# 2gunsu/monocon-pytorch

Measured on AMD Instinct MI355X. Metric: images/sec (384x1280) fwd+bwd, higher is better.
Workload: dtype f32 (f16x2); 1 GPU; train step B=32/GPU 3x384x1280 (configs[2] shape, fp32 values, mode f16x2); global_batch=32, parallelism=dp1, precision_mode=f16x2

## Files before the change

### monocon-pytorch_amd/csrc/conv_thin.hip

```cpp
#include "conv_mfma.h"
#include "train.h"

#ifndef THIN_OCC
#define THIN_OCC 2
#endif
#ifndef THIN_MT_UNROLL
#define THIN_MT_UNROLL 1
#endif
namespace mc {

typedef _Float16 f16x8 __attribute__((ext_vector_type(8)));
typedef _Float16 f16x4 __attribute__((ext_vector_type(4)));
typedef float f32x4v __attribute__((ext_vector_type(4)));

namespace {
constexpr int TR = 8, TW = 64;
constexpr int IR = TR + 2, IP = TW + 2;
constexpr int PLANE = IR * IP * 16;
constexpr int ITEMS = IR * IP * 4;
constexpr int NI = (ITEMS + 255) / 256;
}

template <int NTN>
__global__ __launch_bounds__(256, THIN_OCC) void conv_thin16_kernel(const ConvArgs a) {
    constexpr int CIN = 16;
    __shared__ __attribute__((aligned(16))) unsigned char lds[4 * PLANE];
    const int tid = threadIdx.x, lane = tid & 63;
    const int wave = __builtin_amdgcn_readfirstlane(tid >> 6);
    const int li = lane & 15, kq = lane >> 4;
    const int half = kq & 1, tsel = kq >> 1;

    const int ex = f16_scale_exp(amax_read(a.amax_in[0])), ew = f16_scale_exp(*a.amax_w);
    const float x_scale = exp2i(ex), w_scale = exp2i(ew);
    const float omul = exp2i(-ex) * exp2i(-ew);
    const bool lazy = a.src[0].la != nullptr;
    f32x4 lzA = {0.f, 0.f, 0.f, 0.f}, lzB = lzA;
    if (lazy) {
        lzA = reinterpret_cast<const f32x4 *>(a.src[0].la)[tid & 3];
        lzB = reinterpret_cast<const f32x4 *>(a.src[0].lb)[tid & 3];
#pragma unroll
        for (int j = 0; j < 4; ++j) { lzA[j] *= x_scale; lzB[j] *= x_scale; }
    }
    const unsigned x_bytes = (unsigned)(a.Hin * a.Win * CIN) * 4u;
    unsigned okm = 0u;

    f16x8 bw[5][2][NTN];
#pragma unroll
    for (int s = 0; s < 5; ++s) {
        const int tap = 2 * s + tsel;
#pragma unroll
        for (int nt = 0; nt < NTN; ++nt) {
            f16x8 h8, l8;
#pragma unroll
            for (int c4 = 0; c4 < 2; ++c4) {
                f32x4 w = {0.f, 0.f, 0.f, 0.f};
                if (tap < 9)
                    w = *reinterpret_cast<const f32x4 *>(a.wpk + ((size_t)(tap * (CIN / 4) + half * 2 + c4) * a.CoutP + nt * 16 + li) * 4);
#pragma unroll
                for (int j = 0; j < 4; ++j) {
                    const float ws = w[j] * w_scale;
                    const _Float16 hh = (_Float16)ws;
                    h8[c4 * 4 + j] = hh;
                    l8[c4 * 4 + j] = (_Float16)(ws - (float)hh);
                }
            }
            bw[s][0][nt] = h8;
            bw[s][1][nt] = l8;
        }
    }

    float sc[NTN], bi[NTN], sh[NTN];
    bool nok[NTN];
#pragma unroll
    for (int nt = 0; nt < NTN; ++nt) {
        const int n = nt * 16 + li;
        nok[nt] = n < a.Cout;
        sc[nt] = (a.scale && nok[nt]) ? a.scale[n] : 1.f;
        bi[nt] = (a.bias && nok[nt]) ? a.bias[n] : 0.f;
        sh[nt] = (a.stat_shift && nok[nt]) ? a.stat_shift[n] : 0.f;
    }
    const bool do_stats = a.stats != nullptr, has_res = a.res != nullptr;
    const float floor_v = a.relu ? 0.f : -__builtin_inff();
    float vmax = 0.f;
    const bool bm = a.bm_y != nullptr;
    const int bm_relu = a.bm_relu;
    float ma[NTN], mb[NTN];
#pragma unroll
    for (int nt = 0; nt < NTN; ++nt) {
        ma[nt] = (bm && bm_relu == 2 && nok[nt]) ? a.bm_a[nt * 16 + li] : 0.f;
        mb[nt] = (bm && bm_relu == 2 && nok[nt]) ? a.bm_b[nt * 16 + li] : 0.f;
    }

    int s_off[NI], s_dst[NI];
#pragma unroll
    for (int i = 0; i < NI; ++i) {
        const int e = tid + 256 * i;
        const int c4 = e & 3, px = (e >> 2) % IP, row = (e >> 2) / IP;
        s_off[i] = ((row * a.Win + px) * CIN + c4 * 4) * 4;
        s_dst[i] = e < ITEMS ? ((c4 >> 1) * PLANE) + (row * IP + px) * 16 + (c4 & 1) * 8 : -1;
    }

    const int tiles_per_img = (a.Hout + TR - 1) / TR;
    const int nstrips = (a.Wout + TW - 1) / TW;
    for (int tile = xcd_order(blockIdx.x, gridDim.x); tile < a.B * tiles_per_img; tile += gridDim.x) {
        const int img = tile / tiles_per_img, oy0 = (tile - img * tiles_per_img) * TR;
        const __amdgpu_buffer_rsrc_t r_x = make_rsrc(a.src[0].p + (size_t)img * a.Hin * a.Win * CIN, (unsigned)(a.Hin * a.Win * CIN) * 4u);
        __amdgpu_buffer_rsrc_t r_out[2], r_res[2];
#pragma unroll
        for (int q = 0; q < 2; ++q) {
            const int oy = oy0 + 2 * wave + q;
            const bool ok = oy < a.Hout;
            const size_t row = (size_t)img * a.Hout + (ok ? oy : 0);
            r_out[q] = make_rsrc(a.out + row * a.Wout * a.out_ld, ok ? (unsigned)(a.Wout * a.out_ld) * 4u : 0u);
            r_res[q] = make_rsrc(has_res ? a.res + row * a.Wout * a.res_ld : a.out, (has_res && ok) ? (unsigned)(a.Wout * a.res_ld) * 4u : 0u);
        }
        float ssum[2][NTN], ssq[2][NTN];
#pragma unroll
        for (int q = 0; q < 2; ++q)
#pragma unroll
            for (int nt = 0; nt < NTN; ++nt) ssum[q][nt] = ssq[q][nt] = 0.f;

        f32x4 pre[NI];
        const int band_off = ((oy0 - 1) * a.Win - 1) * CIN * 4;
        auto fetch = [&](int strip) {
            const int x0 = strip * TW - 1, so = band_off + strip * TW * CIN * 4;
            okm = 0u;
            if (strip > 0 && x0 + IP <= a.Win) {
#pragma unroll
                for (int i = 0; i < NI; ++i) {
                    const int vo = s_dst[i] >= 0 ? s_off[i] + so : BUF_OOB;
                    pre[i] = buf_load4(r_x, vo, 0);
                    if (lazy) okm |= ((unsigned)vo < x_bytes ? 1u : 0u) << i;
                }
            } else {
#pragma unroll
                for (int i = 0; i < NI; ++i) {
                    const int px = ((s_dst[i] % PLANE) >> 4) % IP;
                    const bool ok = s_dst[i] >= 0 && (unsigned)(x0 + px) < (unsigned)a.Win;
                    const int vo = ok ? s_off[i] + so : BUF_OOB;
                    pre[i] = buf_load4(r_x, vo, 0);
                    if (lazy) okm |= ((unsigned)vo < x_bytes ? 1u : 0u) << i;
                }
            }
        };
        auto store = [&]() {
#pragma unroll
            for (int i = 0; i < NI; ++i) {
                if (256 * (i + 1) > ITEMS && s_dst[i] < 0) continue;
                f16x4 h4, l4;
                const float cap = ((okm >> i) & 1u) ? __builtin_inff() : 0.f;
#pragma unroll
                for (int j = 0; j < 4; ++j) {
                    const float xs = lazy ? lazy_act(pre[i][j], lzA[j], lzB[j], cap) : pre[i][j] * x_scale;
                    const _Float16 hh = (_Float16)xs;
                    h4[j] = hh;
                    l4[j] = (_Float16)(xs - (float)hh);
                }
                *reinterpret_cast<f16x4 *>(lds + s_dst[i]) = h4;
                *reinterpret_cast<f16x4 *>(lds + 2 * PLANE + s_dst[i]) = l4;
            }
        };

        fetch(0);
        for (int strip = 0; strip < nstrips; ++strip) {
            __syncthreads();
            store();
            __syncthreads();
            if (strip + 1 < nstrips) fetch(strip + 1);
            const int sx0 = strip * TW;
#pragma unroll
            for (int q = 0; q < 2; ++q) {
                const int trow = 2 * wave + q;
#pragma unroll THIN_MT_UNROLL
                for (int mt = 0; mt < TW / 16; ++mt) {
                    const int x0 = sx0 + mt * 16;
                    if (x0 >= a.Wout) break;
                    f32x4v acc[NTN], accm[NTN];
#pragma unroll
                    for (int nt = 0; nt < NTN; ++nt) { acc[nt] = f32x4v{0.f, 0.f, 0.f, 0.f}; accm[nt] = f32x4v{0.f, 0.f, 0.f, 0.f}; }
                    const bool rok = oy0 + trow < a.Hout;
                    float ybm[NTN][4], zbm[NTN][4];
                    if (bm) {
#pragma unroll
                        for (int nt = 0; nt < NTN; ++nt) {
                            const size_t at0 = (((size_t)img * a.Hout + (rok ? oy0 + trow : 0)) * a.Wout + x0 + 4 * kq) * a.Cout + nt * 16 + li;
#pragma unroll
                            for (int e = 0; e < 4; ++e) {
                                const bool ld = rok && nok[nt];
                                ybm[nt][e] = ld ? a.bm_y[at0 + (size_t)e * a.Cout] : 0.f;
                                zbm[nt][e] = (ld && bm_relu == 1) ? a.bm_z[at0 + (size_t)e * a.Cout] : 1.f;
                            }
                        }
                    }
#pragma unroll
                    for (int s = 0; s < 5; ++s) {
                        const int tap = 2 * s + tsel;
                        const int r = tap / 3, c = tap - 3 * r;
                        f16x8 ah = {0, 0, 0, 0, 0, 0, 0, 0}, al = ah;
                        if (tap < 9) {
                            const unsigned char *p = lds + half * PLANE + ((trow + r) * IP + mt * 16 + li + c) * 16;
                            ah = *reinterpret_cast<const f16x8 *>(p);
                            al = *reinterpret_cast<const f16x8 *>(p + 2 * PLANE);
                        }
#pragma unroll
                        for (int nt = 0; nt < NTN; ++nt) {
                            accm[nt] = __builtin_amdgcn_mfma_f32_16x16x32_f16(al, bw[s][0][nt], accm[nt], 0, 0, 0);
                            accm[nt] = __builtin_amdgcn_mfma_f32_16x16x32_f16(ah, bw[s][1][nt], accm[nt], 0, 0, 0);
                            acc[nt] = __builtin_amdgcn_mfma_f32_16x16x32_f16(ah, bw[s][0][nt], acc[nt], 0, 0, 0);
                        }
                    }
#pragma unroll
                    for (int nt = 0; nt < NTN; ++nt) {
                        const int n = nt * 16 + li;
                        const int v_out = nok[nt] ? ((4 * kq) * a.out_ld + a.out_coff + n) * 4 : BUF_OOB;
                        const int v_res = nok[nt] ? ((4 * kq) * a.res_ld + n) * 4 : BUF_OOB;
                        float rv[4];
                        if (has_res) {
#pragma unroll
                            for (int e = 0; e < 4; ++e) rv[e] = buf_load1(r_res[q], v_res, (x0 + e) * a.res_ld * 4);
                        }
#pragma unroll
                        for (int e = 0; e < 4; ++e) {
                            float v = ((accm[nt][e] + acc[nt][e]) * omul) * sc[nt] + bi[nt];
                            if (has_res) v += rv[e];
                            if (bm) {
                                if (rok && nok[nt]) {
                                    const float yv = ybm[nt][e];
                                    const bool on = bm_relu == 0 || (bm_relu == 1 ? zbm[nt][e] > 0.f : fmaf(yv, ma[nt], mb[nt]) > 0.f);
                                    v = on ? v : 0.f;
                                    ssum[q][nt] += v;
                                    ssq[q][nt] = fmaf(v, yv, ssq[q][nt]);
                                }
                            } else if (do_stats) {
                                const float d = v - sh[nt];
                                ssum[q][nt] += d;
                                ssq[q][nt] += d * d;
                            }
                            v = fmaxf(v, floor_v);
                            vmax = fmaxf(vmax, (nok[nt] && oy0 + trow < a.Hout) ? fabsf(v) : 0.f);
                            buf_store1(v, r_out[q], v_out, (x0 + e) * a.out_ld * 4);
                        }
                    }
                }
            }
        }
        if (do_stats) {
#pragma unroll
            for (int q = 0; q < 2; ++q) {
                const int oy = oy0 + 2 * wave + q;
                if (oy >= a.Hout) continue;
#pragma unroll
                for (int nt = 0; nt < NTN; ++nt) {
                    float s1 = ssum[q][nt], s2 = ssq[q][nt];
                    s1 += __shfl_xor(s1, 16); s2 += __shfl_xor(s2, 16);
                    s1 += __shfl_xor(s1, 32); s2 += __shfl_xor(s2, 32);
                    if (kq == 0 && nok[nt]) {
                        float *dst = a.stats + (((size_t)img * a.Hout + oy) * a.CoutP + nt * 16 + li) * 2;
                        dst[0] = s1;
                        dst[1] = s2;
                    }
                }
            }
        }
    }
    if (a.amax_out) amax_update_wave(a.amax_out, vmax);
}

bool conv_thin_ok(const ConvArgs &a, int ks, int stride) {
#ifdef MC_NO_CONV_THIN
    return false;
#endif
    return a.prec == 3 && ks == 3 && stride == 1 && a.nsrc == 1 && a.Cin == 16 && a.Cout == 16 && a.amax_in[0] && a.amax_w &&
           a.Wout % 16 == 0 && a.Hout == a.Hin && a.Wout == a.Win && a.CoutP >= 16;
}

hipError_t launch_conv_thin(const ConvArgs &a, hipStream_t st) {
    const int tiles = a.B * ((a.Hout + TR - 1) / TR);
    hipLaunchKernelGGL((conv_thin16_kernel<1>), dim3(tiles < 4096 ? tiles : 4096), dim3(256), 0, st, a);
    return hipGetLastError();
}


struct DgradS2Args {
    const float *dy;
    const float *w;
    float *out;
    int B, H, W, CinTotal, c_off, accumulate;
    const unsigned *amax_dy, *amax_w;
};
namespace {
constexpr int DR = 4, DW = 32;
constexpr int DIR_ = DR + 1, DIP = DW + 1;
constexpr int DPLANE = DIR_ * DIP * 16;
}
template <int KS, int NT>
__global__ __launch_bounds__(256, KS == 1 ? 2 : 1) void dgrad_s2_thin_kernel(const DgradS2Args a) {
    constexpr int CY = 32 * KS, CX = 16 * NT, NOCT = 4 * KS;
    constexpr int DITEMS = DIR_ * DIP * (CY / 4), DNI = (DITEMS + 255) / 256;
    __shared__ __attribute__((aligned(16))) unsigned char lds[2 * NOCT * DPLANE];
    const int tid = threadIdx.x, lane = tid & 63;
    const int wave = __builtin_amdgcn_readfirstlane(tid >> 6);
    const int li = lane & 15, kq = lane >> 4;
    const int nt = wave % NT, row0 = (wave / NT) * NT;
    const int ex = f16_scale_exp(amax_read(a.amax_dy)), ew = f16_scale_exp(*a.amax_w);
    const float x_scale = exp2i(ex), w_scale = exp2i(ew), omul = exp2i(-ex) * exp2i(-ew);
    f16x8 bw[9][KS][2];
// ... 94 lines not shown
                                const int voff = j < a.W ? ((2 * j + px) * CX + 16 * nt + li) * 4 : BUF_OOB;
                                float v = (accm[e] + acc[e]) * omul;
                                if (a.accumulate) v += buf_load1(r_out[rr][py], voff, 0);
                                buf_store1(v, r_out[rr][py], voff, 0);
                            }
                        }
                    }
                }
            }
        }
    }
}
bool dgrad_s2_thin_ok(int prec, int ks, int stride, int dyC, int srcC, int CinTotal, int c_off, const unsigned *amax_dy,
                      const unsigned *amax_w, int H, int W) {
    const bool shape = dyC == 32 && srcC == 16;
    return prec == 3 && ks == 3 && stride == 2 && shape && c_off >= 0 && c_off + srcC <= CinTotal && amax_dy && amax_w &&
           (size_t)H * W * dyC * 4 < (1ull << 31) && (size_t)4 * W * srcC * 4 < (1ull << 31);
}
hipError_t launch_dgrad_s2_thin(const float *dy, int B, int H, int W, int dyC, const float *w_master, int CinTotal, int c_off, float *out,
                                int accumulate, const unsigned *amax_dy, const unsigned *amax_w, hipStream_t st) {
    DgradS2Args a;
    a.dy = dy; a.w = w_master; a.out = out; a.B = B; a.H = H; a.W = W; a.CinTotal = CinTotal; a.c_off = c_off;
    a.accumulate = accumulate; a.amax_dy = amax_dy; a.amax_w = amax_w;
    const int tiles = B * ((H + DR - 1) / DR);
    const int srcC = dyC / 2;
    prof_last = {1, 2.0 * B * H * W * (double)dyC * srcC * 9.0, 4.0 * ((double)B * H * W * dyC + (double)B * 4 * H * W * srcC * (accumulate ? 2 : 1))};
    if (dyC != 32) return hipErrorInvalidValue;
    hipLaunchKernelGGL((dgrad_s2_thin_kernel<1, 1>), dim3(tiles < 4096 ? tiles : 4096), dim3(256), 0, st, a);
    return hipGetLastError();
}

namespace {
constexpr int WT_XT = 128, WT_P = 152, WT_ROWS = 6;
constexpr int WT_PLANE = 16 * WT_ROWS * WT_P * 2;
typedef unsigned u32x4 __attribute__((ext_vector_type(4)));
typedef _Float16 f16x2 __attribute__((ext_vector_type(2)));
}

__global__ __launch_bounds__(256) void wgrad_thin16_kernel(const WgradArgs a) {
    extern __shared__ __attribute__((aligned(16))) unsigned char wsm[];
    unsigned char *win = wsm;
    float (*red)[64] = reinterpret_cast<float (*)[64]>(wsm + 2 * WT_PLANE);
    const int tid = threadIdx.x, lane = tid & 63;
    const int wave = __builtin_amdgcn_readfirstlane(tid >> 6);
    const int g = lane >> 4, j = lane & 15;
    const int ex = f16_scale_exp(amax_read(a.amax_x[0])), ed = f16_scale_exp(amax_read(a.amax_dy));
    const float x_scale = exp2i(ex), d_scale = exp2i(ed), omul = exp2i(-ex) * exp2i(-ed);
    const int H = a.Hout, W = a.Wout;
    const bool lazy = a.src[0].la != nullptr;
    f32x4 lzA = {0.f, 0.f, 0.f, 0.f}, lzB = lzA;
    if (lazy) {
        lzA = reinterpret_cast<const f32x4 *>(a.src[0].la)[tid & 3];
        lzB = reinterpret_cast<const f32x4 *>(a.src[0].lb)[tid & 3];
#pragma unroll
        for (int q = 0; q < 4; ++q) { lzA[q] *= x_scale; lzB[q] *= x_scale; }
    }
    const unsigned x_bytes = (unsigned)(a.Hin * a.Win * 16) * 4u;
    unsigned okm = 0u;

    f32x4v acc[9], accm[9];
#pragma unroll
    for (int t = 0; t < 9; ++t) { acc[t] = f32x4v{0.f, 0.f, 0.f, 0.f}; accm[t] = f32x4v{0.f, 0.f, 0.f, 0.f}; }
    const int va = (8 * g * 16 + j) * 4;
    const int boff = ((j * WT_ROWS + wave) * WT_P + 8 * g) * 2;

    constexpr int NITEM = WT_ROWS * (WT_P / 2) * 4, NIW = (NITEM + 255) / 256;
    int w_off[NIW], w_dst[NIW];
#pragma unroll
    for (int i = 0; i < NIW; ++i) {
        const int e = tid + 256 * i, c4 = e & 3, pr = (e >> 2) % (WT_P / 2), row = (e >> 2) / (WT_P / 2);
        w_off[i] = ((row * a.Win + 2 * pr) * 16 + c4 * 4) * 4;
        w_dst[i] = e < NITEM ? ((c4 * 4 * WT_ROWS + row) * WT_P + 2 * pr) * 2 : -1;
    }
    const int tiles_x = (W + WT_XT - 1) / WT_XT, tiles_y = (H + 3) / 4;
    const int ntiles = a.B * tiles_y * tiles_x;
    f32x4 pv[NIW][2];
    auto fetch = [&](int tl) {
        const int b = tl / (tiles_y * tiles_x), rem = tl - b * tiles_y * tiles_x;
        const int y0 = (rem / tiles_x) * 4, x0 = (rem % tiles_x) * WT_XT;
        const __amdgpu_buffer_rsrc_t r_x = make_rsrc(a.src[0].p + (size_t)b * a.Hin * a.Win * 16, (unsigned)(a.Hin * a.Win * 16) * 4u);
        const int so = ((y0 - 1) * a.Win + x0 - 1) * 64;
        okm = 0u;
#pragma unroll
        for (int i = 0; i < NIW; ++i) {
            const int col = x0 - 1 + ((w_dst[i] >> 1) % WT_P);
            const bool live = w_dst[i] >= 0;
            const int vo0 = (live && col >= 0 && col < a.Win) ? w_off[i] + so : BUF_OOB;
            const int vo1 = (live && col + 1 >= 0 && col + 1 < a.Win) ? w_off[i] + so + 64 : BUF_OOB;
            pv[i][0] = buf_load4(r_x, vo0, 0);
            pv[i][1] = buf_load4(r_x, vo1, 0);
            if (lazy) okm |= (((unsigned)vo0 < x_bytes ? 1u : 0u) | ((unsigned)vo1 < x_bytes ? 2u : 0u)) << (2 * i);
        }
    };
    float araw[WT_XT / 32][8];
    auto fetch_dy = [&](int tl, float (&dst)[WT_XT / 32][8]) {
        const int b = tl / (tiles_y * tiles_x), rem = tl - b * tiles_y * tiles_x;
        const int y = (rem / tiles_x) * 4 + wave, x0 = (rem % tiles_x) * WT_XT;
        const __amdgpu_buffer_rsrc_t r_dy =
            make_rsrc(a.dy + ((size_t)b * H + (y < H ? y : 0)) * W * a.dy_ld, y < H ? (unsigned)(W * a.dy_ld) * 4u : 0u);
#pragma unroll
        for (int G = 0; G < WT_XT / 32; ++G)
#pragma unroll
            for (int t = 0; t < 8; ++t) dst[G][t] = buf_load1(r_dy, va + t * 64, (x0 + G * 32) * 64);
// ... 108 lines not shown
```

### monocon-pytorch_amd/csrc/stem_f16.hip

```cpp
#include "conv_mfma.h"
#include "kernels.h"

#ifndef STEM_MT_UNROLL
#define STEM_MT_UNROLL 1
#endif
namespace mc {

typedef _Float16 f16x8 __attribute__((ext_vector_type(8)));
typedef _Float16 f16x4 __attribute__((ext_vector_type(4)));
typedef float f32x4v __attribute__((ext_vector_type(4)));

namespace {
constexpr int SR = 8, SW = 64;
constexpr int SIR = SR + 6, SIP = 72;
constexpr int SPIX = SIR * SIP;
constexpr int SNI = (SPIX + 255) / 256;
}

__global__ __launch_bounds__(256) void stem_f16_kernel(const float *__restrict__ img, int B, int H, int W,
                                                       const float *__restrict__ wpk ,
                                                       const float *__restrict__ scale, const float *__restrict__ shift,
                                                       float *__restrict__ out, int relu, unsigned *__restrict__ amax_out,
                                                       float *__restrict__ stats ,
                                                       const float *__restrict__ stat_shift,
                                                       unsigned *__restrict__ img_amax ) {
    __shared__ __attribute__((aligned(16))) unsigned char lds[2 * SPIX * 8];
    __shared__ unsigned s_max;
    const int tid = threadIdx.x, lane = tid & 63;
    const int wave = __builtin_amdgcn_readfirstlane(tid >> 6);
    const int li = lane & 15, kq = lane >> 4;
    const int tiles_y = (H + SR - 1) / SR, nstrips = (W + SW - 1) / SW;
    const int bt = xcd_order(blockIdx.x, gridDim.x);
    const int b = bt / tiles_y;
    const int ty0 = (bt % tiles_y) * SR;

    float wv[7][8];
    float wmax = 0.f;
#pragma unroll
    for (int r = 0; r < 7; ++r)
#pragma unroll
        for (int p = 0; p < 2; ++p)
#pragma unroll
            for (int c = 0; c < 4; ++c) {
                const int s = 2 * kq + p;
                const float w = (c < 3 && s < 7) ? wpk[((c * 7 + r) * 7 + s) * 16 + li] : 0.f;
                wv[r][p * 4 + c] = w;
                wmax = fmaxf(wmax, fabsf(w));
            }
#pragma unroll
    for (int o = 32; o > 0; o >>= 1) wmax = fmaxf(wmax, __shfl_xor(wmax, o));
    const int ew = f16_scale_exp(__builtin_bit_cast(unsigned, wmax));
    const float w_scale = exp2i(ew);
    f16x8 bw[7][2];
#pragma unroll
    for (int r = 0; r < 7; ++r)
#pragma unroll
        for (int j = 0; j < 8; ++j) {
            const float ws = wv[r][j] * w_scale;
            const _Float16 hh = (_Float16)ws;
            bw[r][0][j] = hh;
            bw[r][1][j] = (_Float16)(ws - (float)hh);
        }

    const float sc = scale[li], sf = shift[li];
    const float sh = (stats && stat_shift) ? stat_shift[li] : 0.f;
    float vmax = 0.f;
    float ssum[2] = {0.f, 0.f}, ssq[2] = {0.f, 0.f};

    float xin[SNI][3];
    auto fetch = [&](int strip) {
        const int tx0 = strip * SW;
#pragma unroll
        for (int i = 0; i < SNI; ++i) {
            const int e = tid + 256 * i;
            const int ly = e / SIP, lx = e - ly * SIP;
            const int y = ty0 - 3 + ly, x = tx0 - 3 + lx;
            const bool ok = e < SPIX && y >= 0 && y < H && x >= 0 && x < W;
#pragma unroll
            for (int c = 0; c < 3; ++c) xin[i][c] = ok ? img[(((size_t)b * 3 + c) * H + y) * W + x] : 0.f;
        }
    };
    fetch(0);
    for (int strip = 0; strip < nstrips; ++strip) {
        const int tx0 = strip * SW;
        float xmax = 0.f;
#pragma unroll
        for (int i = 0; i < SNI; ++i)
#pragma unroll
            for (int c = 0; c < 3; ++c) xmax = fmaxf(xmax, fabsf(xin[i][c]));
        if (tid == 0) s_max = 0u;
        __syncthreads();
        {
            const unsigned bits = __builtin_bit_cast(unsigned, xmax);
            if (bits != 0u && bits < 0x7f800000u) atomicMax(&s_max, bits);
        }
        __syncthreads();
        const int ex = f16_scale_exp(s_max);
        const float x_scale = exp2i(ex);
        const float omul = exp2i(-ex) * exp2i(-ew);
        if (img_amax && tid == 0) amax_commit(img_amax, s_max);
// ... 1 lines not shown
        for (int i = 0; i < SNI; ++i) {
            const int e = tid + 256 * i;
            if (e >= SPIX) continue;
            f16x4 h4, l4;
#pragma unroll
            for (int c = 0; c < 4; ++c) {
                const float xs = c < 3 ? xin[i][c] * x_scale : 0.f;
                const _Float16 hh = (_Float16)xs;
                h4[c] = hh;
                l4[c] = (_Float16)(xs - (float)hh);
            }
            *reinterpret_cast<f16x4 *>(lds + e * 8) = h4;
            *reinterpret_cast<f16x4 *>(lds + SPIX * 8 + e * 8) = l4;
        }
        __syncthreads();
        if (strip + 1 < nstrips) fetch(strip + 1);
#pragma unroll
        for (int q = 0; q < 2; ++q) {
            const int trow = 2 * wave + q, y = ty0 + trow;
            if (y >= H) continue;
            float *orow = out + ((size_t)b * H + y) * W * 16;
#pragma unroll STEM_MT_UNROLL
            for (int mt = 0; mt < SW / 16; ++mt) {
                const int x0 = tx0 + mt * 16;
                if (x0 >= W) break;
                f32x4v acc = {0.f, 0.f, 0.f, 0.f}, accm = {0.f, 0.f, 0.f, 0.f};
#pragma unroll
                for (int r = 0; r < 7; ++r) {
                    const unsigned char *p = lds + ((trow + r) * SIP + mt * 16 + li + 2 * kq) * 8;
                    const f16x4 h0 = *reinterpret_cast<const f16x4 *>(p), h1 = *reinterpret_cast<const f16x4 *>(p + 8);
                    const f16x4 l0 = *reinterpret_cast<const f16x4 *>(p + SPIX * 8), l1 = *reinterpret_cast<const f16x4 *>(p + SPIX * 8 + 8);
                    const f16x8 ah = {h0[0], h0[1], h0[2], h0[3], h1[0], h1[1], h1[2], h1[3]};
                    const f16x8 al = {l0[0], l0[1], l0[2], l0[3], l1[0], l1[1], l1[2], l1[3]};
                    accm = __builtin_amdgcn_mfma_f32_16x16x32_f16(al, bw[r][0], accm, 0, 0, 0);
                    accm = __builtin_amdgcn_mfma_f32_16x16x32_f16(ah, bw[r][1], accm, 0, 0, 0);
                    acc = __builtin_amdgcn_mfma_f32_16x16x32_f16(ah, bw[r][0], acc, 0, 0, 0);
                }
#pragma unroll
                for (int e = 0; e < 4; ++e) {
                    const int x = x0 + 4 * kq + e;
                    float v = fmaf((accm[e] + acc[e]) * omul, sc, sf);
                    if (relu) v = fmaxf(v, 0.f);
                    if (x < W) {
                        orow[(size_t)x * 16 + li] = v;
                        vmax = fmaxf(vmax, fabsf(v));
                        const float d = v - sh;
                        ssum[q] += d;
                        ssq[q] = fmaf(d, d, ssq[q]);
                    }
                }
            }
        }
    }
    if (stats) {
#pragma unroll
        for (int q = 0; q < 2; ++q) {
            const int y = ty0 + 2 * wave + q;
            float s1 = ssum[q], s2 = ssq[q];
            s1 += __shfl_xor(s1, 16); s2 += __shfl_xor(s2, 16);
            s1 += __shfl_xor(s1, 32); s2 += __shfl_xor(s2, 32);
            if (kq == 0 && y < H) {
                float *dst = stats + (((size_t)b * H + y) * 16 + li) * 2;
                dst[0] = s1;
                dst[1] = s2;
            }
        }
    }
    if (amax_out) amax_update_wave(amax_out, vmax);
}

hipError_t launch_stem_f16(const float *img, int B, int H, int W, const float *wpk, const float *scale, const float *shift,
                           float *out, hipStream_t st, int relu, unsigned *amax_out, float *stats, const float *stat_shift,
                           unsigned *img_amax) {
    const int tiles = (H + SR - 1) / SR;
    hipLaunchKernelGGL(stem_f16_kernel, dim3(B * tiles), dim3(256), 0, st, img, B, H, W, wpk, scale, shift, out, relu, amax_out, stats,
                       stat_shift, img_amax);
    return hipGetLastError();
}


namespace {
constexpr int GW_XT = 128, GW_P = 144, GW_ROWS = 10;
typedef unsigned u32x4 __attribute__((ext_vector_type(4)));
}

template <bool FUSED>
__global__ __launch_bounds__(256) void stem_wgrad_f16_kernel(const float *__restrict__ img, const float *__restrict__ dy, int B,
                                                             int H, int W, float *__restrict__ partial,
                                                             const unsigned *__restrict__ img_amax,
                                                             const unsigned *__restrict__ dy_amax,
                                                             const float *__restrict__ ybn, const float *__restrict__ coef,
                                                             const unsigned *__restrict__ y_amax) {
    constexpr int PLANE_B = 3 * GW_ROWS * GW_P * 2;
    __shared__ __attribute__((aligned(16))) unsigned char win[2 * PLANE_B];
    __shared__ float red[14 * 4][64];
    const int tid = threadIdx.x, lane = tid & 63;
    const int wave = __builtin_amdgcn_readfirstlane(tid >> 6);
    const int g = lane >> 4, j = lane & 15;
    float cP = 0.f, cQ = 0.f, cR = 0.f;
    int ed;
    if constexpr (FUSED) {
        const f32x4v cf = reinterpret_cast<const f32x4v *>(coef)[j];
        cP = cf[0]; cQ = cf[1]; cR = cf[2];
        float mP = fabsf(cP), mQ = fabsf(cQ), mR = fabsf(cR);
#pragma unroll
        for (int o = 8; o > 0; o >>= 1) {
            mP = fmaxf(mP, __shfl_xor(mP, o)); mQ = fmaxf(mQ, __shfl_xor(mQ, o)); mR = fmaxf(mR, __shfl_xor(mR, o));
        }
        const float bound = mP * __builtin_bit_cast(float, amax_read(dy_amax)) + mQ * __builtin_bit_cast(float, amax_read(y_amax)) + mR;
        ed = f16_scale_exp(__builtin_bit_cast(unsigned, bound));
    } else {
        ed = f16_scale_exp(amax_read(dy_amax));
    }
    const int ex = f16_scale_exp(amax_read(img_amax));
    const float x_scale = exp2i(ex), d_scale = exp2i(ed), omul = exp2i(-ex) * exp2i(-ed);
    int boff[2];
#pragma unroll
    for (int grp = 0; grp < 2; ++grp) {
        const int cr = grp * 16 + j, c = cr / 7, r = cr - 7 * c;
        boff[grp] = cr < 21 ? ((c * GW_ROWS + wave + r) * GW_P + 8 * g) * 2 : 0;
    }
    f32x4v acc[2][7], accm[2][7];
#pragma unroll
    for (int grp = 0; grp < 2; ++grp)
#pragma unroll
        for (int sft = 0; sft < 7; ++sft) { acc[grp][sft] = f32x4v{0.f, 0.f, 0.f, 0.f}; accm[grp][sft] = f32x4v{0.f, 0.f, 0.f, 0.f}; }
    const int va = (8 * g * 16 + j) * 4;
    const int tiles_x = (W + GW_XT - 1) / GW_XT, tiles_y = (H + 3) / 4;
    const int ntiles = B * tiles_y * tiles_x;
    constexpr int NPAIR = 3 * GW_ROWS * (GW_P / 2), NIW = (NPAIR + 255) / 256;
    int w_c[NIW], w_rr[NIW], w_col[NIW];
#pragma unroll
    for (int i = 0; i < NIW; ++i) {
        const int e = tid + 256 * i, row = e / (GW_P / 2);
        w_c[i] = e < NPAIR ? row / GW_ROWS : -1;
        w_rr[i] = row % GW_ROWS;
        w_col[i] = (e - row * (GW_P / 2)) * 2;
    }
    float pv[NIW][2];
    auto fetch = [&](int tl) {
        const int b = tl / (tiles_y * tiles_x), rem = tl - b * tiles_y * tiles_x;
        const int y0 = (rem / tiles_x) * 4, x0 = (rem % tiles_x) * GW_XT;
#pragma unroll
        for (int i = 0; i < NIW; ++i) {
            const int gy = y0 - 3 + w_rr[i], gx = x0 - 3 + w_col[i];
            const bool rok = w_c[i] >= 0 && gy >= 0 && gy < H;
            const float *src = img + (((size_t)b * 3 + (rok ? w_c[i] : 0)) * H + (rok ? gy : 0)) * W;
            pv[i][0] = (rok && gx >= 0 && gx < W) ? src[gx] : 0.f;
            pv[i][1] = (rok && gx + 1 >= 0 && gx + 1 < W) ? src[gx + 1] : 0.f;
        }
    };
    if ((int)blockIdx.x < ntiles) fetch(blockIdx.x);
    for (int tl = blockIdx.x; tl < ntiles; tl += gridDim.x) {
        const int b = tl / (tiles_y * tiles_x), rem = tl - b * tiles_y * tiles_x;
        const int y0 = (rem / tiles_x) * 4, x0 = (rem % tiles_x) * GW_XT;
        __syncthreads();
#pragma unroll
        for (int i = 0; i < NIW; ++i) {
            if (w_c[i] < 0) continue;
            const float s0 = pv[i][0] * x_scale, s1 = pv[i][1] * x_scale;
            const _Float16 h0 = (_Float16)s0, h1 = (_Float16)s1;
            typedef _Float16 f16x2 __attribute__((ext_vector_type(2)));
            const f16x2 hp = {h0, h1}, lp = {(_Float16)(s0 - (float)h0), (_Float16)(s1 - (float)h1)};
            const int off = ((w_c[i] * GW_ROWS + w_rr[i]) * GW_P + w_col[i]) * 2;
            *reinterpret_cast<f16x2 *>(win + off) = hp;
            *reinterpret_cast<f16x2 *>(win + PLANE_B + off) = lp;
        }
        __syncthreads();
        if (tl + (int)gridDim.x < ntiles) fetch(tl + gridDim.x);
        const int y = y0 + wave;
// ... 99 lines not shown
```

Before: 678.4 images/sec.

## Transpose MFMA operands in thin16/stem convs for vectorized 128-bit epilogue stores

Swaps the A/B operands of the MFMA calls in the thin 16-channel conv and the stem conv, so each lane's accumulator holds 4 consecutive output channels of one pixel instead of 4 pixels of one channel. The epilogue can then use a single 128-bit buffer store and load per tile for output, residual and backward-mask inputs, replacing four scalar strided accesses. Per-channel scale, bias and stat accumulators become 4-wide, and the stats reduction moves to a 16-lane shuffle tree. The change also trims the wgrad window fetch to the columns actually used, raises stem occupancy via launch bounds, and adds alignment guards on out_ld, out_coff and res_ld. It costs more registers for the per-channel vectors and extra shuffles in the stats reduction.

```diff
diff --git a/monocon-pytorch_amd/csrc/conv_thin.hip b/monocon-pytorch_amd/csrc/conv_thin.hip
--- a/monocon-pytorch_amd/csrc/conv_thin.hip
+++ b/monocon-pytorch_amd/csrc/conv_thin.hip
@@ -14,6 +14,9 @@
 typedef float f32x4v __attribute__((ext_vector_type(4)));
 
 namespace {
+__device__ __forceinline__ void buf_store4(f32x4 v, __amdgpu_buffer_rsrc_t r, int voff, int soff) {
+    __builtin_amdgcn_raw_buffer_store_b128(__builtin_bit_cast(i32x4, v), r, voff, soff, 0);
+}
 constexpr int TR = 8, TW = 64;
 constexpr int IR = TR + 2, IP = TW + 2;
 constexpr int PLANE = IR * IP * 16;
@@ -69,27 +72,32 @@
         }
     }
 
-    float sc[NTN], bi[NTN], sh[NTN];
+    float sc[NTN][4], bi[NTN][4], sh[NTN][4];
     bool nok[NTN];
 #pragma unroll
     for (int nt = 0; nt < NTN; ++nt) {
-        const int n = nt * 16 + li;
-        nok[nt] = n < a.Cout;
-        sc[nt] = (a.scale && nok[nt]) ? a.scale[n] : 1.f;
-        bi[nt] = (a.bias && nok[nt]) ? a.bias[n] : 0.f;
-        sh[nt] = (a.stat_shift && nok[nt]) ? a.stat_shift[n] : 0.f;
+        const int n0 = nt * 16 + 4 * kq;
+        nok[nt] = n0 + 3 < a.Cout;
+#pragma unroll
+        for (int e = 0; e < 4; ++e) {
+            sc[nt][e] = (a.scale && nok[nt]) ? a.scale[n0 + e] : 1.f;
+            bi[nt][e] = (a.bias && nok[nt]) ? a.bias[n0 + e] : 0.f;
+            sh[nt][e] = (a.stat_shift && nok[nt]) ? a.stat_shift[n0 + e] : 0.f;
+        }
     }
     const bool do_stats = a.stats != nullptr, has_res = a.res != nullptr;
     const float floor_v = a.relu ? 0.f : -__builtin_inff();
     float vmax = 0.f;
     const bool bm = a.bm_y != nullptr;
     const int bm_relu = a.bm_relu;
-    float ma[NTN], mb[NTN];
-#pragma unroll
-    for (int nt = 0; nt < NTN; ++nt) {
-        ma[nt] = (bm && bm_relu == 2 && nok[nt]) ? a.bm_a[nt * 16 + li] : 0.f;
-        mb[nt] = (bm && bm_relu == 2 && nok[nt]) ? a.bm_b[nt * 16 + li] : 0.f;
-    }
+    float ma[NTN][4], mb[NTN][4];
+#pragma unroll
+    for (int nt = 0; nt < NTN; ++nt)
+#pragma unroll
+        for (int e = 0; e < 4; ++e) {
+            ma[nt][e] = (bm && bm_relu == 2 && nok[nt]) ? a.bm_a[nt * 16 + 4 * kq + e] : 0.f;
+            mb[nt][e] = (bm && bm_relu == 2 && nok[nt]) ? a.bm_b[nt * 16 + 4 * kq + e] : 0.f;
+        }
 
     int s_off[NI], s_dst[NI];
 #pragma unroll
@@ -114,11 +122,11 @@
             r_out[q] = make_rsrc(a.out + row * a.Wout * a.out_ld, ok ? (unsigned)(a.Wout * a.out_ld) * 4u : 0u);
             r_res[q] = make_rsrc(has_res ? a.res + row * a.Wout * a.res_ld : a.out, (has_res && ok) ? (unsigned)(a.Wout * a.res_ld) * 4u : 0u);
         }
-        float ssum[2][NTN], ssq[2][NTN];
+        f32x4 ssum[2][NTN], ssq[2][NTN];
 #pragma unroll
         for (int q = 0; q < 2; ++q)
 #pragma unroll
-            for (int nt = 0; nt < NTN; ++nt) ssum[q][nt] = ssq[q][nt] = 0.f;
+            for (int nt = 0; nt < NTN; ++nt) ssum[q][nt] = ssq[q][nt] = f32x4{0.f, 0.f, 0.f, 0.f};
 
         f32x4 pre[NI];
         const int band_off = ((oy0 - 1) * a.Win - 1) * CIN * 4;
@@ -179,17 +187,14 @@
 #pragma unroll
                     for (int nt = 0; nt < NTN; ++nt) { acc[nt] = f32x4v{0.f, 0.f, 0.f, 0.f}; accm[nt] = f32x4v{0.f, 0.f, 0.f, 0.f}; }
                     const bool rok = oy0 + trow < a.Hout;
-                    float ybm[NTN][4], zbm[NTN][4];
+                    f32x4 ybm[NTN], zbm[NTN];
                     if (bm) {
 #pragma unroll
                         for (int nt = 0; nt < NTN; ++nt) {
-                            const size_t at0 = (((size_t)img * a.Hout + (rok ? oy0 + trow : 0)) * a.Wout + x0 + 4 * kq) * a.Cout + nt * 16 + li;
-#pragma unroll
-                            for (int e = 0; e < 4; ++e) {
-                                const bool ld = rok && nok[nt];
-                                ybm[nt][e] = ld ? a.bm_y[at0 + (size_t)e * a.Cout] : 0.f;
-                                zbm[nt][e] = (ld && bm_relu == 1) ? a.bm_z[at0 + (size_t)e * a.Cout] : 1.f;
-                            }
+                            const size_t at0 = (((size_t)img * a.Hout + (rok ? oy0 + trow : 0)) * a.Wout + x0 + li) * a.Cout + nt * 16 + 4 * kq;
+                            const bool ld = rok && nok[nt];
+                            ybm[nt] = ld ? *reinterpret_cast<const f32x4 *>(a.bm_y + at0) : f32x4{0.f, 0.f, 0.f, 0.f};
+                            zbm[nt] = (ld && bm_relu == 1) ? *reinterpret_cast<const f32x4 *>(a.bm_z + at0) : f32x4{1.f, 1.f, 1.f, 1.f};
                         }
                     }
 #pragma unroll
@@ -204,42 +209,40 @@
                         }
 #pragma unroll
                         for (int nt = 0; nt < NTN; ++nt) {
-                            accm[nt] = __builtin_amdgcn_mfma_f32_16x16x32_f16(al, bw[s][0][nt], accm[nt], 0, 0, 0);
-                            accm[nt] = __builtin_amdgcn_mfma_f32_16x16x32_f16(ah, bw[s][1][nt], accm[nt], 0, 0, 0);
-                            acc[nt] = __builtin_amdgcn_mfma_f32_16x16x32_f16(ah, bw[s][0][nt], acc[nt], 0, 0, 0);
+                            accm[nt] = __builtin_amdgcn_mfma_f32_16x16x32_f16(bw[s][0][nt], al, accm[nt], 0, 0, 0);
+                            accm[nt] = __builtin_amdgcn_mfma_f32_16x16x32_f16(bw[s][1][nt], ah, accm[nt], 0, 0, 0);
+                            acc[nt] = __builtin_amdgcn_mfma_f32_16x16x32_f16(bw[s][0][nt], ah, acc[nt], 0, 0, 0);
                         }
                     }
 #pragma unroll
                     for (int nt = 0; nt < NTN; ++nt) {
-                        const int n = nt * 16 + li;
-                        const int v_out = nok[nt] ? ((4 * kq) * a.out_ld + a.out_coff + n) * 4 : BUF_OOB;
-                        const int v_res = nok[nt] ? ((4 * kq) * a.res_ld + n) * 4 : BUF_OOB;
-                        float rv[4];
-                        if (has_res) {
-#pragma unroll
-                            for (int e = 0; e < 4; ++e) rv[e] = buf_load1(r_res[q], v_res, (x0 + e) * a.res_ld * 4);
-                        }
+                        const int n0 = nt * 16 + 4 * kq;
+                        const int v_out = nok[nt] ? (li * a.out_ld + a.out_coff + n0) * 4 : BUF_OOB;
+                        const int v_res = nok[nt] ? (li * a.res_ld + n0) * 4 : BUF_OOB;
+                        f32x4 rv = {0.f, 0.f, 0.f, 0.f}, o;
+                        if (has_res) rv = buf_load4(r_res[q], v_res, x0 * a.res_ld * 4);
 #pragma unroll
                         for (int e = 0; e < 4; ++e) {
-                            float v = ((accm[nt][e] + acc[nt][e]) * omul) * sc[nt] + bi[nt];
+                            float v = ((accm[nt][e] + acc[nt][e]) * omul) * sc[nt][e] + bi[nt][e];
                             if (has_res) v += rv[e];
                             if (bm) {
                                 if (rok && nok[nt]) {
                                     const float yv = ybm[nt][e];
-                                    const bool on = bm_relu == 0 || (bm_relu == 1 ? zbm[nt][e] > 0.f : fmaf(yv, ma[nt], mb[nt]) > 0.f);
+                                    const bool on = bm_relu == 0 || (bm_relu == 1 ? zbm[nt][e] > 0.f : fmaf(yv, ma[nt][e], mb[nt][e]) > 0.f);
                                     v = on ? v : 0.f;
-                                    ssum[q][nt] += v;
-                                    ssq[q][nt] = fmaf(v, yv, ssq[q][nt]);
+                                    ssum[q][nt][e] += v;
+                                    ssq[q][nt][e] = fmaf(v, yv, ssq[q][nt][e]);
                                 }
                             } else if (do_stats) {
-                                const float d = v - sh[nt];
-                                ssum[q][nt] += d;
-                                ssq[q][nt] += d * d;
+                                const float d = v - sh[nt][e];
+                                ssum[q][nt][e] += d;
+                                ssq[q][nt][e] += d * d;
                             }
                             v = fmaxf(v, floor_v);
                             vmax = fmaxf(vmax, (nok[nt] && oy0 + trow < a.Hout) ? fabsf(v) : 0.f);
-                            buf_store1(v, r_out[q], v_out, (x0 + e) * a.out_ld * 4);
+                            o[e] = v;
                         }
+                        buf_store4(o, r_out[q], v_out, x0 * a.out_ld * 4);
                     }
                 }
             }
@@ -251,13 +254,16 @@
                 if (oy >= a.Hout) continue;
 #pragma unroll
                 for (int nt = 0; nt < NTN; ++nt) {
-                    float s1 = ssum[q][nt], s2 = ssq[q][nt];
-                    s1 += __shfl_xor(s1, 16); s2 += __shfl_xor(s2, 16);
-                    s1 += __shfl_xor(s1, 32); s2 += __shfl_xor(s2, 32);
-                    if (kq == 0 && nok[nt]) {
-                        float *dst = a.stats + (((size_t)img * a.Hout + oy) * a.CoutP + nt * 16 + li) * 2;
-                        dst[0] = s1;
-                        dst[1] = s2;
+#pragma unroll
+                    for (int e = 0; e < 4; ++e) {
+                        float s1 = ssum[q][nt][e], s2 = ssq[q][nt][e];
+#pragma unroll
+                        for (int o = 1; o < 16; o <<= 1) { s1 += __shfl_xor(s1, o); s2 += __shfl_xor(s2, o); }
+                        if (li == 0 && nok[nt]) {
+                            float *dst = a.stats + (((size_t)img * a.Hout + oy) * a.CoutP + nt * 16 + 4 * kq + e) * 2;
+                            dst[0] = s1;
+                            dst[1] = s2;
+                        }
                     }
                 }
             }
@@ -271,7 +277,8 @@
     return false;
 #endif
     return a.prec == 3 && ks == 3 && stride == 1 && a.nsrc == 1 && a.Cin == 16 && a.Cout == 16 && a.amax_in[0] && a.amax_w &&
-           a.Wout % 16 == 0 && a.Hout == a.Hin && a.Wout == a.Win && a.CoutP >= 16;
+           a.Wout % 16 == 0 && a.Hout == a.Hin && a.Wout == a.Win && a.CoutP >= 16 &&
+           a.out_ld % 4 == 0 && a.out_coff % 4 == 0 && (!a.res || a.res_ld % 4 == 0);
 }
 
 hipError_t launch_conv_thin(const ConvArgs &a, hipStream_t st) {
@@ -432,6 +439,7 @@
 
 namespace {
 constexpr int WT_XT = 128, WT_P = 152, WT_ROWS = 6;
+constexpr int WT_USED = 130;
 constexpr int WT_PLANE = 16 * WT_ROWS * WT_P * 2;
 typedef unsigned u32x4 __attribute__((ext_vector_type(4)));
 typedef _Float16 f16x2 __attribute__((ext_vector_type(2)));
@@ -464,11 +472,11 @@
     const int va = (8 * g * 16 + j) * 4;
     const int boff = ((j * WT_ROWS + wave) * WT_P + 8 * g) * 2;
 
-    constexpr int NITEM = WT_ROWS * (WT_P / 2) * 4, NIW = (NITEM + 255) / 256;
+    constexpr int NITEM = WT_ROWS * (WT_USED / 2) * 4, NIW = (NITEM + 255) / 256;
     int w_off[NIW], w_dst[NIW];
 #pragma unroll
     for (int i = 0; i < NIW; ++i) {
-        const int e = tid + 256 * i, c4 = e & 3, pr = (e >> 2) % (WT_P / 2), row = (e >> 2) / (WT_P / 2);
+        const int e = tid + 256 * i, c4 = e & 3, pr = (e >> 2) % (WT_USED / 2), row = (e >> 2) / (WT_USED / 2);
         w_off[i] = ((row * a.Win + 2 * pr) * 16 + c4 * 4) * 4;
         w_dst[i] = e < NITEM ? ((c4 * 4 * WT_ROWS + row) * WT_P + 2 * pr) * 2 : -1;
     }
diff --git a/monocon-pytorch_amd/csrc/stem_f16.hip b/monocon-pytorch_amd/csrc/stem_f16.hip
--- a/monocon-pytorch_amd/csrc/stem_f16.hip
+++ b/monocon-pytorch_amd/csrc/stem_f16.hip
@@ -17,7 +17,7 @@
 constexpr int SNI = (SPIX + 255) / 256;
 }
 
-__global__ __launch_bounds__(256) void stem_f16_kernel(const float *__restrict__ img, int B, int H, int W,
+__global__ __launch_bounds__(256, 3) void stem_f16_kernel(const float *__restrict__ img, int B, int H, int W,
                                                        const float *__restrict__ wpk ,
                                                        const float *__restrict__ scale, const float *__restrict__ shift,
                                                        float *__restrict__ out, int relu, unsigned *__restrict__ amax_out,
@@ -62,10 +62,17 @@
             bw[r][1][j] = (_Float16)(ws - (float)hh);
         }
 
-    const float sc = scale[li], sf = shift[li];
-    const float sh = (stats && stat_shift) ? stat_shift[li] : 0.f;
+    f32x4v sc, sf, sh;
+#pragma unroll
+    for (int e = 0; e < 4; ++e) {
+        sc[e] = scale[4 * kq + e];
+        sf[e] = shift[4 * kq + e];
+        sh[e] = (stats && stat_shift) ? stat_shift[4 * kq + e] : 0.f;
+    }
     float vmax = 0.f;
-    float ssum[2] = {0.f, 0.f}, ssq[2] = {0.f, 0.f};
+    f32x4v ssum[2], ssq[2];
+#pragma unroll
+    for (int q = 0; q < 2; ++q) ssum[q] = ssq[q] = f32x4v{0.f, 0.f, 0.f, 0.f};
 
     float xin[SNI][3];
     auto fetch = [&](int strip) {
@@ -133,22 +140,24 @@
                     const f16x4 l0 = *reinterpret_cast<const f16x4 *>(p + SPIX * 8), l1 = *reinterpret_cast<const f16x4 *>(p + SPIX * 8 + 8);
                     const f16x8 ah = {h0[0], h0[1], h0[2], h0[3], h1[0], h1[1], h1[2], h1[3]};
                     const f16x8 al = {l0[0], l0[1], l0[2], l0[3], l1[0], l1[1], l1[2], l1[3]};
-                    accm = __builtin_amdgcn_mfma_f32_16x16x32_f16(al, bw[r][0], accm, 0, 0, 0);
-                    accm = __builtin_amdgcn_mfma_f32_16x16x32_f16(ah, bw[r][1], accm, 0, 0, 0);
-                    acc = __builtin_amdgcn_mfma_f32_16x16x32_f16(ah, bw[r][0], acc, 0, 0, 0);
-                }
-#pragma unroll
-                for (int e = 0; e < 4; ++e) {
-                    const int x = x0 + 4 * kq + e;
-                    float v = fmaf((accm[e] + acc[e]) * omul, sc, sf);
-                    if (relu) v = fmaxf(v, 0.f);
-                    if (x < W) {
-                        orow[(size_t)x * 16 + li] = v;
+                    accm = __builtin_amdgcn_mfma_f32_16x16x32_f16(bw[r][0], al, accm, 0, 0, 0);
+                    accm = __builtin_amdgcn_mfma_f32_16x16x32_f16(bw[r][1], ah, accm, 0, 0, 0);
+                    acc = __builtin_amdgcn_mfma_f32_16x16x32_f16(bw[r][0], ah, acc, 0, 0, 0);
+                }
+                const int x = x0 + li;
+                if (x < W) {
+                    f32x4v o;
+#pragma unroll
+                    for (int e = 0; e < 4; ++e) {
+                        float v = fmaf((accm[e] + acc[e]) * omul, sc[e], sf[e]);
+                        if (relu) v = fmaxf(v, 0.f);
+                        o[e] = v;
                         vmax = fmaxf(vmax, fabsf(v));
-                        const float d = v - sh;
-                        ssum[q] += d;
-                        ssq[q] = fmaf(d, d, ssq[q]);
+                        const float d = v - sh[e];
+                        ssum[q][e] += d;
+                        ssq[q][e] = fmaf(d, d, ssq[q][e]);
                     }
+                    *reinterpret_cast<f32x4v *>(orow + (size_t)x * 16 + 4 * kq) = o;
                 }
             }
         }
@@ -157,13 +166,16 @@
 #pragma unroll
         for (int q = 0; q < 2; ++q) {
             const int y = ty0 + 2 * wave + q;
-            float s1 = ssum[q], s2 = ssq[q];
-            s1 += __shfl_xor(s1, 16); s2 += __shfl_xor(s2, 16);
-            s1 += __shfl_xor(s1, 32); s2 += __shfl_xor(s2, 32);
-            if (kq == 0 && y < H) {
-                float *dst = stats + (((size_t)b * H + y) * 16 + li) * 2;
-                dst[0] = s1;
-                dst[1] = s2;
+#pragma unroll
+            for (int e = 0; e < 4; ++e) {
+                float s1 = ssum[q][e], s2 = ssq[q][e];
+#pragma unroll
+                for (int o = 1; o < 16; o <<= 1) { s1 += __shfl_xor(s1, o); s2 += __shfl_xor(s2, o); }
+                if (li == 0 && y < H) {
+                    float *dst = stats + (((size_t)b * H + y) * 16 + 4 * kq + e) * 2;
+                    dst[0] = s1;
+                    dst[1] = s2;
+                }
             }
         }
     }
@@ -182,6 +194,7 @@
 
 namespace {
 constexpr int GW_XT = 128, GW_P = 144, GW_ROWS = 10;
+constexpr int GW_USED = 134;
 typedef unsigned u32x4 __attribute__((ext_vector_type(4)));
 }
 
@@ -229,14 +242,14 @@
     const int va = (8 * g * 16 + j) * 4;
     const int tiles_x = (W + GW_XT - 1) / GW_XT, tiles_y = (H + 3) / 4;
     const int ntiles = B * tiles_y * tiles_x;
-    constexpr int NPAIR = 3 * GW_ROWS * (GW_P / 2), NIW = (NPAIR + 255) / 256;
+    constexpr int NPAIR = 3 * GW_ROWS * (GW_USED / 2), NIW = (NPAIR + 255) / 256;
     int w_c[NIW], w_rr[NIW], w_col[NIW];
 #pragma unroll
     for (int i = 0; i < NIW; ++i) {
-        const int e = tid + 256 * i, row = e / (GW_P / 2);
+        const int e = tid + 256 * i, row = e / (GW_USED / 2);
         w_c[i] = e < NPAIR ? row / GW_ROWS : -1;
         w_rr[i] = row % GW_ROWS;
-        w_col[i] = (e - row * (GW_P / 2)) * 2;
+        w_col[i] = (e - row * (GW_USED / 2)) * 2;
     }
     float pv[NIW][2];
     auto fetch = [&](int tl) {
diff --git a/scratch/front_end/compare_dumps.py b/scratch/front_end/compare_dumps.py
--- /dev/null
+++ b/scratch/front_end/compare_dumps.py
@@ -0,0 +1,16 @@
+import glob
+import os
+import sys
+import numpy as np
+
+new, old, f32 = sys.argv[1:4]
+bad = 0
+print("%-44s %12s %12s" % ("array (relative L2)", "change-parent", "parent-fp32"))
+for f in sorted(glob.glob(os.path.join(old, "*.npy"))):
+    n = os.path.basename(f)
+    a, b, c = (np.load(os.path.join(d, n)).astype(np.float64) for d in (new, old, f32))
+    s = max(float(np.linalg.norm(b)), 1e-30)
+    d1, d2 = float(np.linalg.norm(a - b)) / s, float(np.linalg.norm(b - c)) / s
+    bad += d1 > d2
+    print("%-44s %12.3e %12.3e %s" % (n[:-4], d1, d2, "EXCEEDS" if d1 > d2 else ""))
+sys.exit(1 if bad else 0)
diff --git a/scratch/front_end/make_variants.py b/scratch/front_end/make_variants.py
--- /dev/null
+++ b/scratch/front_end/make_variants.py
@@ -0,0 +1,74 @@
+import os
+import shutil
+import subprocess
+import sys
+import tempfile
+
+HERE = os.path.dirname(os.path.abspath(__file__))
+CSRC = os.path.join(HERE, "..", "..", "monocon-pytorch_amd", "csrc")
+MFMA3 = ("accm{i} = __builtin_amdgcn_mfma_f32_16x16x32_f16({a}l, {b}0, accm{i}, 0, 0, 0);",)
+
+
+def sub(text, old, new, count=None):
+    n = text.count(old)
+    assert n >= 1 and (count is None or n == count), (old, n)
+    return text.replace(old, new)
+
+
+def variant(name, thin, stem):
+    if name == "noload":
+        thin = sub(thin, "pre[i] = buf_load4(r_x, vo, 0);", "pre[i] = f32x4{1.f, 1.f, 1.f, 1.f};", 2)
+        thin = sub(thin, "pv[i][0] = buf_load4(r_x, vo0, 0);", "pv[i][0] = f32x4{1.f, 1.f, 1.f, 1.f};", 1)
+        thin = sub(thin, "pv[i][1] = buf_load4(r_x, vo1, 0);", "pv[i][1] = f32x4{1.f, 1.f, 1.f, 1.f};", 1)
+        stem = sub(stem, "xin[i][c] = ok ? img[(((size_t)b * 3 + c) * H + y) * W + x] : 0.f;", "xin[i][c] = ok ? 1.f : 0.f;", 1)
+        stem = sub(stem, "araw[G][t] = buf_load1(r_dy, va + t * 64, (x0 + G * 32) * 64);", "araw[G][t] = 1.f;", 1)
+        stem = sub(stem, "yraw[G][t] = buf_load1(r_y, va + t * 64, (x0 + G * 32) * 64);", "yraw[G][t] = 1.f;", 1)
+    elif name == "nody":
+        thin = sub(thin, "dst[G][t] = buf_load1(r_dy, va + t * 64, (x0 + G * 32) * 64);", "dst[G][t] = 1.f;", 1)
+        stem = sub(stem, "pv[i][0] = (rok && gx >= 0 && gx < W) ? src[gx] : 0.f;", "pv[i][0] = rok ? 1.f : 0.f;", 1)
+        stem = sub(stem, "pv[i][1] = (rok && gx + 1 >= 0 && gx + 1 < W) ? src[gx + 1] : 0.f;", "pv[i][1] = rok ? 1.f : 0.f;", 1)
+    elif name == "nomfma":
+        for a, b in (("__builtin_amdgcn_mfma_f32_16x16x32_f16(bw[s][0][nt], al, accm[nt], 0, 0, 0)", "accm[nt] + (float)al[0]"),
+                     ("__builtin_amdgcn_mfma_f32_16x16x32_f16(bw[s][1][nt], ah, accm[nt], 0, 0, 0)", "accm[nt] + (float)ah[1]"),
+                     ("__builtin_amdgcn_mfma_f32_16x16x32_f16(bw[s][0][nt], ah, acc[nt], 0, 0, 0)", "acc[nt] + (float)ah[0] * (float)bw[s][0][nt][0]"),
+                     ("__builtin_amdgcn_mfma_f32_16x16x32_f16(al, bh, accm[t], 0, 0, 0)", "accm[t] + (float)al[0]"),
+                     ("__builtin_amdgcn_mfma_f32_16x16x32_f16(ah, bl, accm[t], 0, 0, 0)", "accm[t] + (float)bl[0]"),
+                     ("__builtin_amdgcn_mfma_f32_16x16x32_f16(ah, bh, acc[t], 0, 0, 0)", "acc[t] + (float)ah[0] * (float)bh[sft]")):
+            thin = sub(thin, a, b, 1)
+        for a, b in (("__builtin_amdgcn_mfma_f32_16x16x32_f16(bw[r][0], al, accm, 0, 0, 0)", "accm + (float)al[0]"),
+                     ("__builtin_amdgcn_mfma_f32_16x16x32_f16(bw[r][1], ah, accm, 0, 0, 0)", "accm + (float)ah[1]"),
+                     ("__builtin_amdgcn_mfma_f32_16x16x32_f16(bw[r][0], ah, acc, 0, 0, 0)", "acc + (float)ah[0] * (float)bw[r][0][0]"),
+                     ("__builtin_amdgcn_mfma_f32_16x16x32_f16(al, bh, accm[grp][sft], 0, 0, 0)", "accm[grp][sft] + (float)al[0]"),
+                     ("__builtin_amdgcn_mfma_f32_16x16x32_f16(ah, bl, accm[grp][sft], 0, 0, 0)", "accm[grp][sft] + (float)bl[0]"),
+                     ("__builtin_amdgcn_mfma_f32_16x16x32_f16(ah, bh, acc[grp][sft], 0, 0, 0)", "acc[grp][sft] + (float)ah[0] * (float)bh[sft]")):
+            stem = sub(stem, a, b, 1)
+    elif name == "nostore":
+        thin = sub(thin, "buf_store4(o, r_out[q], v_out, x0 * a.out_ld * 4);", "", 1)
+        stem = sub(stem, "*reinterpret_cast<f32x4v *>(orow + (size_t)x * 16 + 4 * kq) = o;", "", 1)
+    else:
+        raise SystemExit("unknown variant " + name)
+    return thin, stem
+
+
+def main():
+    names = sys.argv[1:] or ["noload", "nody", "nomfma", "nostore"]
+    out = os.path.join(HERE, "variants")
+    os.makedirs(out, exist_ok=True)
+    for name in names:
+        tmp = tempfile.mkdtemp(prefix="fe_" + name + "_")
+        dst = os.path.join(tmp, "monocon-pytorch_amd", "csrc")
+        shutil.copytree(CSRC, dst, ignore=shutil.ignore_patterns("*.o"))
+        shutil.copytree(os.path.join(CSRC, "..", "..", "include"), os.path.join(tmp, "include"))
+        for f in os.listdir(CSRC):
+            if f.endswith(".o") and f not in ("conv_thin.o", "stem_f16.o"):
+                shutil.copy2(os.path.join(CSRC, f), dst)
+        thin, stem = variant(name, open(os.path.join(dst, "conv_thin.hip")).read(), open(os.path.join(dst, "stem_f16.hip")).read())
+        open(os.path.join(dst, "conv_thin.hip"), "w").write(thin)
+        open(os.path.join(dst, "stem_f16.hip"), "w").write(stem)
+        subprocess.check_call(["make", "-C", dst, "-j2", "LIB=" + os.path.join(out, "lib_%s.so" % name)])
+        shutil.rmtree(tmp)
+        print("built", name)
+
+
+if __name__ == "__main__":
+    main()
diff --git a/scratch/front_end/pick_seed.py b/scratch/front_end/pick_seed.py
--- /dev/null
+++ b/scratch/front_end/pick_seed.py
@@ -0,0 +1,58 @@
+import os
+import sys
+import numpy as np
+import torch
+
+REPO = os.path.dirname(os.path.dirname(os.path.dirname(os.path.abspath(__file__))))
+sys.path[:0] = [os.path.join(REPO, "monocon-pytorch_amd"), REPO, os.path.join(REPO, "tests")]
+from hipmonocon import synth, netspec
+from oracle import monocon_oracle as O
+
+
+def grads(sd, batch, f64):
+    live = {}
+    for k, v in sd.items():
+        if v.dtype == torch.float32:
+            v = v.double() if f64 else v.clone()
+            live[k] = v.clone().requires_grad_(True) if "running" not in k else v.clone()
+        else:
+            live[k] = v.clone()
+    b = dict(batch)
+    b["img"] = batch["img"].double() if f64 else batch["img"].float()
+    _, _, L, _ = O.train_forward(live, b)
+    sum(L.values()).backward()
+    return {k: p.grad.double() for k, p in live.items() if getattr(p, "grad", None) is not None}
+
+
+FRONT = ("backbone.base_layer.0.weight", "backbone.base_layer.1.weight", "backbone.base_layer.1.bias", "backbone.level0.0.weight")
+
+
+def errs(a, b):
+    out = {}
+    for k in FRONT:
+        scale = max(float(b[k].norm()), 1e-30)
+        out[k] = float((a[k] - b[k]).norm() / scale)
+    return out
+
+
+B, H, W = (int(x) for x in sys.argv[1:4])
+seed = int(sys.argv[4]) if len(sys.argv) > 4 else 500
+stats = np.load(os.path.join(REPO, "tests", "golden", "bn_calib_seed7.npz"))
+sd = synth.make_conditioned_state_dict(7, bn_stats={k: stats[k] for k in stats.files})
+for _ in range(300):
+    seed += 1
+    b = synth.make_conditioned_batch(seed, B, H, W)
+    g64 = grads(sd, b, True)
+    noise = torch.from_numpy(synth.uniform(seed, "cond.noise", tuple(b["img"].shape), -1.0, 1.0))
+    bp = dict(b)
+    bp["img"] = b["img"].double() * (1.0 + 3e-7 * noise)
+    em = max(errs(grads(sd, bp, True), g64).values())
+    if em >= 1e-4:
+        print("seed %d rejected: perturbed-fp64 max %.1e" % (seed, em), flush=True)
+        continue
+    e32 = max(errs(grads(sd, b, False), g64).values())
+    if e32 >= 2e-4:
+        print("seed %d rejected: fp32 max %.1e" % (seed, e32), flush=True)
+        continue
+    print("PICKED seed %d B=%d %dx%d: perturbed-fp64 %.1e, oracle fp32-vs-fp64 %.1e" % (seed, B, H, W, em, e32), flush=True)
+    break
diff --git a/scratch/front_end/stats_rows.py b/scratch/front_end/stats_rows.py
--- /dev/null
+++ b/scratch/front_end/stats_rows.py
@@ -0,0 +1,10 @@
+import csv
+import glob
+import sys
+
+for f in sorted(glob.glob(sys.argv[1] + "/**/*kernel_stats.csv", recursive=True)):
+    for r in csv.DictReader(open(f)):
+        n = r["Name"]
+        if any(k in n for k in ("thin16", "stem_f16", "stem_wgrad_f16", "dgrad_s2_thin", "affine_bwd", "chan_reduce")):
+            print("%-60s calls %4s  avg %9.1f us  min %9.1f  max %9.1f  total %9.3f ms" % (
+                n[:60], r["Calls"], float(r["AverageNs"]) / 1e3, float(r["MinNs"]) / 1e3, float(r["MaxNs"]) / 1e3, float(r["TotalDurationNs"]) / 1e6))
diff --git a/scratch/front_end/time_ops.py b/scratch/front_end/time_ops.py
--- /dev/null
+++ b/scratch/front_end/time_ops.py
@@ -0,0 +1,43 @@
+import os
+import sys
+import torch
+
+REPO = os.path.dirname(os.path.dirname(os.path.dirname(os.path.abspath(__file__))))
+sys.path[:0] = [os.path.join(REPO, "monocon-pytorch_amd"), REPO]
+from hipmonocon.engine import Engine
+
+iters = int(sys.argv[1]) if len(sys.argv) > 1 else 10
+B, H, W = 32, 384, 1280
+g = torch.Generator(device="cuda").manual_seed(1)
+eng = Engine()
+eng.set_precision(3)
+x = torch.randn((B, H, W, 16), device="cuda", generator=g)
+dy = torch.randn((B, H, W, 16), device="cuda", generator=g)
+img = torch.randn((B, 3, H, W), device="cuda", generator=g)
+w = torch.randn((16, 16, 3, 3), device="cuda", generator=g) * 0.1
+ws = torch.randn((16, 3, 7, 7), device="cuda", generator=g) * 0.1
+sc = torch.ones(16, device="cuda")
+bi = torch.zeros(16, device="cuda")
+
+
+def timed(name, fn):
+    for _ in range(2):
+        fn()
+    torch.cuda.synchronize()
+    ts = []
+    for _ in range(iters):
+        e0, e1 = torch.cuda.Event(enable_timing=True), torch.cuda.Event(enable_timing=True)
+        e0.record()
+        fn()
+        e1.record()
+        torch.cuda.synchronize()
+        ts.append(e0.elapsed_time(e1) * 1e3)
+    ts.sort()
+    print("%-28s op time us: min %.0f median %.0f max %.0f  (the op = the kernel + its small helpers)" % (name, ts[0], ts[len(ts) // 2], ts[-1]), flush=True)
+
+
+timed("op_stem", lambda: eng.op_stem(img, ws, sc, bi))
+timed("op_conv 16->16 relu", lambda: eng.op_conv([x], w, 1, None, bi, None, True))
+timed("op_conv 16->16 res relu", lambda: eng.op_conv([x], w, 1, None, bi, dy, True))
+timed("op_conv_wgrad 16->16", lambda: eng.op_conv_wgrad([x], dy, 3, 1))
+eng.close()
```

Result: no change. 679.2 images/sec, median of 3 (+0.1%).
